# Orion-AI-Lab/KuroSiwo

Hardware: AMD Instinct MI355X
Metric: SAR tiles/sec (224x224, SNUNet-ECAM change-detection train step) (higher is better)
Workload: dtype bf16; 1 GPU; BASELINE.json configs[1]: SNUNet-ECAM CD, 2 dates x 2-ch GRD 224x224, per-GPU batch 32, ce+dice loss, Adam lr 1e-3, fwd+loss+bwd+optimizer; global_batch=32, base_channel=32, parallelism=dp1, hip_streams=3

## Files before the change

include/ksmi.h:

```cpp
#ifndef KSMI_H
#define KSMI_H
#include <stddef.h>
#include <stdint.h>

#ifdef __cplusplus
extern "C" {
#endif

#define KSMI_ABI_VERSION 8
#define KSMI_F32 0
#define KSMI_BF16 1
#define KSMI_E_ARG (-1)
#define KSMI_E_UNSUPPORTED (-2)
#define KSMI_MAX_SRC 6
#define KSMI_MAX_CHUNKS 72

int ksmi_abi_version(void);
const char* ksmi_last_error(void);
int ksmi_set_knob(const char* name, const char* value);
int ksmi_chunk_elems(int dtype);

#define KSMI_OP_CALL 0
#define KSMI_OP_ORDER 1
#define KSMI_OP_WAIT_SIDE 2
// ... 28 lines not shown
  int32_t C;
  int32_t c_off;
  int32_t n_begin;
  int32_t n_len;
  int32_t accumulate;
  int32_t pad_;
} ksmi_dst;

typedef struct ksmi_conv_desc {
  ksmi_src src[KSMI_MAX_SRC];
  ksmi_dst dst[KSMI_MAX_SRC];
  int32_t nsrc, ndst;
  const void* wpk;
  const float* bias;
  float* stats;
  const void* mask_src;
  const float* m_mean; const float* m_rstd; const float* m_scale; const float* m_shift;
  int32_t B, Hin, Win, Hout, Wout;
  int32_t KH, KW, stride, pad;
  int32_t TH, TW;
  int32_t N, Npad;
  int32_t nchunks;
  int32_t ps_cout;
  uint16_t chunk_c0[KSMI_MAX_CHUNKS];
  uint8_t chunk_src[KSMI_MAX_CHUNKS];
  int32_t pad_x;
  int32_t out_sy, out_sx, out_oy, out_ox, out_H, out_W;
  int32_t uniform_kc;
  int32_t in_sy, in_sx, in_oy, in_ox, in_H, in_W;
  float alpha;
  int32_t relu_out;
  int32_t residC;
  const void* resid;
  int32_t stats_rows;
  const void* gate_src; const void* xhat_src; const float* g_mean; const float* g_rstd;
  int32_t dir;
  int32_t pad2_;
} ksmi_conv_desc;


int ksmi_last_kernels(char* buf, int cap);
int ksmi_hbm_probe(int mode, const void* a, void* b, void* c, size_t nbytes, unsigned* sink, void* stream);
size_t ksmi_desc_size(int which);
int ksmi_conv_gate_supported(const ksmi_conv_desc* d, int dtype);
int ksmi_conv_grid_m(const ksmi_conv_desc* d);
int ksmi_conv_stats_rows(const ksmi_conv_desc* d, int dtype);
// ... 370 lines not shown
```

kurosiwo_amd/_lib.py:

```python
import ctypes as C
import os

_HERE = os.path.dirname(os.path.abspath(__file__))
LIB_PATH = os.path.join(_HERE, "libksmi.so")

KSMI_F32, KSMI_BF16 = 0, 1
LOSS_DICE, LOSS_LOVASZ, LOSS_FOCAL = 1, 2, 3
MAX_SRC, MAX_CHUNKS = 6, 72
ABI_VERSION = 8


class KsmiError(RuntimeError):
    pass


class Src(C.Structure):
    _fields_ = [("ptr", C.c_void_p), ("scale", C.c_void_p), ("shift", C.c_void_p),
                ("C", C.c_int32), ("c_off", C.c_int32), ("c_len", C.c_int32), ("relu", C.c_int32)]


class Dst(C.Structure):
    _fields_ = [("ptr", C.c_void_p), ("C", C.c_int32), ("c_off", C.c_int32), ("n_begin", C.c_int32),
                ("n_len", C.c_int32), ("accumulate", C.c_int32), ("pad_", C.c_int32)]


class ConvDesc(C.Structure):
    _fields_ = [("src", Src * MAX_SRC), ("dst", Dst * MAX_SRC), ("nsrc", C.c_int32), ("ndst", C.c_int32),
                ("wpk", C.c_void_p), ("bias", C.c_void_p), ("stats", C.c_void_p),
                ("mask_src", C.c_void_p), ("m_mean", C.c_void_p), ("m_rstd", C.c_void_p),
                ("m_scale", C.c_void_p), ("m_shift", C.c_void_p),
                ("B", C.c_int32), ("Hin", C.c_int32), ("Win", C.c_int32), ("Hout", C.c_int32), ("Wout", C.c_int32),
                ("KH", C.c_int32), ("KW", C.c_int32), ("stride", C.c_int32), ("pad", C.c_int32),
                ("TH", C.c_int32), ("TW", C.c_int32), ("N", C.c_int32), ("Npad", C.c_int32),
                ("nchunks", C.c_int32), ("ps_cout", C.c_int32),
                ("chunk_c0", C.c_uint16 * MAX_CHUNKS), ("chunk_src", C.c_uint8 * MAX_CHUNKS),
                ("pad_x", C.c_int32), ("out_sy", C.c_int32), ("out_sx", C.c_int32), ("out_oy", C.c_int32),
                ("out_ox", C.c_int32), ("out_H", C.c_int32), ("out_W", C.c_int32),
                ("uniform_kc", C.c_int32), ("in_sy", C.c_int32), ("in_sx", C.c_int32), ("in_oy", C.c_int32), ("in_ox", C.c_int32),
                ("in_H", C.c_int32), ("in_W", C.c_int32), ("alpha", C.c_float), ("relu_out", C.c_int32), ("residC", C.c_int32),
                ("resid", C.c_void_p), ("stats_rows", C.c_int32),
                ("gate_src", C.c_void_p), ("xhat_src", C.c_void_p), ("g_mean", C.c_void_p), ("g_rstd", C.c_void_p),
                ("dir", C.c_int32), ("pad2_", C.c_int32)]


class PackDesc(C.Structure):
    _fields_ = [("w", C.c_void_p), ("out", C.c_void_p),
                ("nchunks", C.c_int32), ("taps", C.c_int32), ("N", C.c_int32), ("Npad", C.c_int32), ("n_mod", C.c_int32),
                ("sK", C.c_int64), ("sN", C.c_int64), ("sD", C.c_int64), ("sT", C.c_int64),
                ("flip", C.c_int32),
                ("k_off", C.c_int32 * MAX_CHUNKS), ("k_len", C.c_int32 * MAX_CHUNKS),
                ("use_tap_map", C.c_int32), ("tap_map", C.c_int32 * 16), ("uniform_kc", C.c_int32), ("k_total", C.c_int32)]


class TiffInfo(C.Structure):
    _fields_ = [(k, C.c_int32) for k in ("width", "height", "bands", "bits", "sample_format", "compression", "predictor", "tiled",
                                         "big_endian", "bigtiff", "has_geo", "has_nodata")] + [
        ("pixel_scale", C.c_double * 2), ("origin", C.c_double * 2), ("tie_pixel", C.c_double * 2), ("nodata", C.c_double)]
# ... 292 lines not shown
```

kurosiwo_amd/csrc/conv_api.hip:

```cpp
#include <stdint.h>
#include "../../include/ksmi.h"
#include "errors.h"
#include "igemm1.h"
#include "igemm3.h"
#include "igemm4.h"
#include "wgrad3.h"

namespace {

enum RowsRule { ROWS_AS_SET, ROWS_OF_KERNEL };
struct ConvRoute { int gen; ksmi_igemm3_geom_t g3; ksmi_igemm4_geom_t g4; };

ConvRoute conv_route(const ksmi_conv_desc* d, int dtype, RowsRule rule) {
  static const bool force_v1 = ksmi_knob_is_set("KSMI_IGEMM_V1");
  ConvRoute r = {};
  r.gen = 1;
  if (force_v1) return r;
  auto rows_ok = [&](int gx) { return rule == ROWS_OF_KERNEL || d->stats == nullptr || d->stats_rows == gx; };
  if (!d->gate_src && ksmi_igemm3_geom(d, dtype, &r.g3) && rows_ok(r.g3.gx)) r.gen = 3;
  else if (ksmi_igemm4_geom(d, dtype, &r.g4) && rows_ok(r.g4.gx)) r.gen = 4;
  else if (ksmi_igemm2_eligible(d, dtype)) r.gen = 2;
  return r;
}

ConvRoute conv_route_with_stats(const ksmi_conv_desc* d, int dtype, bool gate) {
  ksmi_conv_desc c = *d;
  if (!c.stats) c.stats = (float*)(uintptr_t)16;
  if (gate && !c.gate_src) { c.gate_src = (const void*)(uintptr_t)16; c.xhat_src = c.gate_src; c.g_mean = (const float*)(uintptr_t)16; c.g_rstd = c.g_mean; }
  return conv_route(&c, dtype, ROWS_OF_KERNEL);
}

enum { CORE_PATCH = 1, CORE_TOKEN1 = 2, CORE_GEMM2 = 3, CORE_WGRAD3 = 4 };
struct WgradRoute {
  int core, reducer;
  int bias;
  bool plain, direct;
  int nsplit;
  ksmi_igemm1_wgeom_t g1;
  int rps, bt;
  ksmi_wgrad3_geom_t g3;
};

bool token_eligible(const ksmi_wgrad_desc* d, int dtype) {
  static const bool generic = ksmi_knob_is_set("KSMI_WGRAD_GENERIC");
  return dtype == KSMI_BF16 && d->KH == 1 && d->KW == 1 && d->stride == 1 && d->pad == 0 && d->nsrc == 1 && d->src[0].scale == nullptr &&
         d->Hin == d->Hout && d->Win == d->Wout && (d->src[0].c_len % 8) == 0 && (d->N % 8) == 0 && d->N >= 64 && d->src[0].c_len >= 64 && !generic;
}

WgradRoute wgrad_route(const ksmi_wgrad_desc* d, int dtype) {
  WgradRoute r = {};
  ksmi_igemm1_wgrad_geom(d, dtype, &r.g1);
// ... 125 lines not shown
```

kurosiwo_amd/csrc/igemm4.hip:

```cpp
#include <stdlib.h>
#include <type_traits>
#include "common.h"
#include "../../include/ksmi.h"
#include "errors.h"
#include "igemm_epilogue.h"
#include "igemm4.h"
#include "dma.h"

namespace {

template <int N> __device__ __forceinline__ void vm_wait_c() {
  static_assert(N >= 0 && N < 64, "vmcnt field");
  asm volatile("s_waitcnt vmcnt(%0)" ::"n"(N) : "memory");
}

__device__ __attribute__((aligned(64))) unsigned char ig4_zero_page[64];
KSMI_DEVICE_SYMBOL_GETTER(ig4_zero, ig4_zero_page)

struct Ig4Args {
  ksmi_conv_desc d;
  uint32_t m_tw, m_hw, m_tx, m_ty;
  int th, tw;
  int hslot, nh, nhs;
  int tiles, gx, gy;
  int rot;
  int stagger;
  int dbg;
  const unsigned char* zero;
};

constexpr int IG4_NHMAX = 5;

__device__ __forceinline__ int swz_h(int hx) { return ((hx >> 2) & 1) << 1; }

template <int WM, int NF, bool AFF, int EPI, bool DBG = false, int DIR = 0, int ROT = 0, int NWV = 8, int KH = 3, int KW = 3>
__global__ __launch_bounds__(64 * NWV, NWV == 4 ? 2 : 1) void igemm4_kernel(const Ig4Args ka) {
  typedef bf16_t T;
  constexpr bool MASK = EPI == 1, GATE = EPI == 2;
  const ksmi_conv_desc& d = ka.d;
  constexpr int NT = 64 * NWV;
  constexpr int WN = NWV / WM;
  constexpr int BNW = 16 * NF;
  constexpr int BN = WN * BNW;
  constexpr int NG = NF / 2;
  static_assert((KH == 3 && KW == 3) || (KH == 2 && KW == 2 && ROT == 3), "taps");
  constexpr int WSLOT = KW * BN * 64;
  constexpr int WPIECES = WSLOT / 1024;
  constexpr int WK = (WPIECES + NWV - 1) / NWV;
  constexpr int NHM = NWV == 4 ? 6 : (WM == 4 ? 3 : IG4_NHMAX);
  constexpr int HSLOT = NHM * NT * 16;
  constexpr int nh = NHM;
  constexpr bool CHUNK = ROT == 3;
  constexpr int NHS = (NWV == 4 || (WM == 8 && NF == 4) || (CHUNK && WM == 8)) ? 2 : 3;
  constexpr bool DEEP = ROT == 2;
  static_assert(!DEEP || (!AFF && !DBG && NHS == 3 && NWV == 8 && BN <= 64), "deep weight ring: 32 / 64-column tiles with three halo slots");
  static_assert(!CHUNK || (!AFF && !DBG && NWV == 8 && (NF == 2 || KH == 2)), "chunk-granular schedule: the NF = 2 tiles and the 2 x 2 phase convolutions");
  constexpr int NWS = CHUNK ? 2 * KH : (DEEP ? 5 : 3);
  constexpr int nhs = NHS;
  extern __shared__ __attribute__((aligned(16))) unsigned char smem[];

  const int tid = threadIdx.x, lane = tid & 63;
// ... 162 lines not shown
  if (tid < BN) bias_tab[tid] = (d.bias && n0 + tid < d.N) ? d.bias[n0 + tid] : 0.f;
  const bool want_stats = d.stats != nullptr;
  const bool late = ka.stagger && wave >= NWV / 2;
  constexpr int LA = NHS - 1;

  auto tile_epilogue = [&](int t, f32x4 (&acc)[4][NF]) {
      {
        int b, oy0, ox0;
        tile_origin(t, b, oy0, ox0);
        uint32_t opix[4];
        bool okp[4];
#pragma unroll
        for (int mf = 0; mf < 4; ++mf) {
          const int p = wm * 64 + mf * 16 + l15;
          const int ly = dTW.div(p), lx = p - ly * TW;
          const int oy = oy0 + ly, ox = ox0 + lx;
          okp[mf] = p < P && oy < d.Hout && ox < d.Wout;
          opix[mf] = (KH != 2 || d.out_sy == 0) ? (uint32_t)((b * d.Hout + oy) * d.Wout + ox)
                                                : (uint32_t)((b * d.out_H + (oy * d.out_sy + d.out_oy)) * d.out_W + (ox * d.out_sx + d.out_ox));
        }
#pragma unroll
        for (int gi = 0; gi < NG; ++gi) {
          const int nc = n0 + (wn * NG + gi) * 32 + g * 8;
          const bool nv = nc < d.N;
          T* const obase = (T*)d.dst[0].ptr + d.dst[0].c_off + nc;
          const T* const mbase = (const T*)d.mask_src + nc;
          float bias8[8], ssum[8], ssq[8];
          {
            const f32x4 a = *(const f32x4*)(bias_tab + (wn * NG + gi) * 32 + g * 8), c = *(const f32x4*)(bias_tab + (wn * NG + gi) * 32 + g * 8 + 4);
#pragma unroll
            for (int j = 0; j < 4; ++j) { bias8[j] = a[j]; bias8[4 + j] = c[j]; }
#pragma unroll
            for (int j = 0; j < 8; ++j) { ssum[j] = 0.f; ssq[j] = 0.f; }
          }
          float mm[(MASK || GATE) ? 8 : 1], mr[(MASK || GATE) ? 8 : 1], mg[MASK ? 8 : 1], mb[MASK ? 8 : 1];
          if constexpr (MASK || GATE) {
            auto ld8 = [&](const float* qp, float* o, int at) {
              const f32x4 a = *(const f32x4*)(qp + at), c = *(const f32x4*)(qp + at + 4);
#pragma unroll
              for (int j = 0; j < 4; ++j) { o[j] = a[j]; o[4 + j] = c[j]; }
            };
#pragma unroll
            for (int j = 0; j < 8; ++j) { mm[j] = 0.f; mr[j] = 0.f; }
            if constexpr (MASK) {
#pragma unroll
              for (int j = 0; j < 8; ++j) { mg[j] = 0.f; mb[j] = 0.f; }
              if (nv) { ld8(d.m_mean, mm, nc); ld8(d.m_rstd, mr, nc); ld8(d.m_scale, mg, nc); ld8(d.m_shift, mb, nc); }
            } else {
              if (nv) { ld8(d.g_mean, mm, nc); ld8(d.g_rstd, mr, nc); }
            }
          }
#pragma unroll
          for (int mh = 0; mh < 4; mh += 2) {
            u32x4 mv[2], zv[2], ov[2];
#pragma unroll
            for (int u = 0; u < 2; ++u) {
              const int mf = mh + u;
              mv[u] = (u32x4){0u, 0u, 0u, 0u}; zv[u] = mv[u]; ov[u] = mv[u];
              if constexpr (MASK) { if (nv && okp[mf]) mv[u] = *(const u32x4*)(mbase + (size_t)opix[mf] * d.N); }
              if constexpr (EPI == 0) { if (has_resid && nv && okp[mf]) mv[u] = *(const u32x4*)((const T*)d.resid + nc + (size_t)opix[mf] * d.residC); }
              if constexpr (GATE) {
                if (nv && okp[mf]) {
                  mv[u] = *(const u32x4*)((const T*)d.gate_src + nc + (size_t)opix[mf] * d.N);
                  zv[u] = *(const u32x4*)((const T*)d.xhat_src + nc + (size_t)opix[mf] * d.N);
                }
              }
              if (accum && nv && okp[mf]) ov[u] = *(const u32x4*)(obase + (size_t)opix[mf] * dC);
            }
#pragma unroll
            for (int u = 0; u < 2; ++u) {
              const int mf = mh + u;
              const bool ok = nv && okp[mf];
              float v[8];
#pragma unroll
              for (int r = 0; r < 4; ++r) { v[r] = acc[mf][2 * gi][r] + bias8[r]; v[4 + r] = acc[mf][2 * gi + 1][r] + bias8[4 + r]; }
              if constexpr (EPI == 0) {
                float rs[8];
                vec_unpack<T>(mv[u], rs);
#pragma unroll
                for (int j = 0; j < 8; ++j) {
                  v[j] = v[j] * alpha + rs[j];
                  if (relu_out) v[j] = fmaxf(v[j], 0.f);
                }
              }
              if constexpr (GATE) {
                float o[8], m[8], z[8];
                vec_unpack<T>(ov[u], o); vec_unpack<T>(mv[u], m); vec_unpack<T>(zv[u], z);
#pragma unroll
                for (int j = 0; j < 8; ++j) {
                  if (accum) v[j] += o[j];
                  if (!(m[j] > 0.f)) v[j] = 0.f;
                }
                const u32x4 pk = vec_pack<T>(v);
                float vr[8];
                vec_unpack<T>(pk, vr);
#pragma unroll
                for (int j = 0; j < 8; ++j) if (ok) { ssum[j] += vr[j]; ssq[j] += vr[j] * ((z[j] - mm[j]) * mr[j]); }
                if (ok && !(DBG && (dbg & 4))) *(u32x4*)(obase + (size_t)opix[mf] * dC) = pk;
              } else {
                if constexpr (MASK) {
                  float m[8];
                  vec_unpack<T>(mv[u], m);
#pragma unroll
                  for (int j = 0; j < 8; ++j) {
                    const float xh = (m[j] - mm[j]) * mr[j];
                    if (!(m[j] * mg[j] + mb[j] > 0.f)) v[j] = 0.f;
                    const float q = ElemTraits<T>::cvt(v[j]);
                    if (ok) { ssum[j] += q; ssq[j] += q * xh; }
                  }
                } else {
                  float q[8];
                  vec_unpack<T>(vec_pack<T>(v), q);
#pragma unroll
                  for (int j = 0; j < 8; ++j) if (ok) { ssum[j] += q[j]; ssq[j] += q[j] * q[j]; }
                }
                if (accum) {
                  float o[8];
                  vec_unpack<T>(ov[u], o);
#pragma unroll
                  for (int j = 0; j < 8; ++j) v[j] += o[j];
                }
// ... 447 lines not shown
      const int hp = (th + 2) * (tw + 2);
      if (hp > hmax) continue;
      const int tiles = ((H + th - 1) / th) * ((W + tw - 1) / tw);
      const double cost = (double)tiles * pmax * (1.0 + 0.15 * hp / pmax);
      if (cost < best) { best = cost; bth = th; btw = tw; }
    }
  *th_o = bth; *tw_o = btw;
}
}

bool ksmi_igemm4_geom(const ksmi_conv_desc* d, int dtype, ksmi_igemm4_geom_t* g) {
  static const bool off = ksmi_knob_is_set("KSMI_IGEMM4_OFF");
  if (off || dtype != KSMI_BF16) return false;
  static const int k2_on = ksmi_knob_int("KSMI_IG4_K2", 1);
  const bool k2 = d->KH == 2 && d->KW == 2;
  if (k2) {
    if (!k2_on || d->stride != 1 || (unsigned)d->pad > 1u || (unsigned)d->pad_x > 1u) return false;
    if (d->Npad % 128 || d->src[0].scale || d->gate_src || (d->out_sy && (d->mask_src || d->dst[0].accumulate))) return false;
    if (d->alpha != 0.f || d->resid || d->relu_out) return false;
  } else if (d->KH != 3 || d->KW != 3 || d->stride != 1 || d->pad != 1 || d->pad_x != 1) return false;
  if (d->Hin != d->Hout || d->Win != d->Wout) return false;
  if (d->nchunks < 2) return false;
  if (d->nchunks > KSMI_MAX_CHUNKS) return false;
  if (d->ndst != 1 || d->dst[0].n_begin != 0) return false;
  if (((d->out_sy || d->in_sy) && !k2) || d->ps_cout) return false;
  if (d->out_sy && ((size_t)d->B * d->out_H * d->out_W >= ((size_t)1 << 31))) return false;
  if ((d->alpha != 0.f || d->resid || d->relu_out) && (d->mask_src || d->gate_src)) return false;
  if (d->resid && (((uintptr_t)d->resid & 15) || (d->residC % 8))) return false;
  if ((d->dst[0].C % 8) || (d->dst[0].c_off % 8)) return false;
  static const int thin_on = ksmi_knob_int("KSMI_IG4_THIN", 1);
  if ((d->N % 8) && (!thin_on || k2 || d->mask_src || d->gate_src || d->resid || d->dst[0].accumulate || d->alpha != 0.f || d->relu_out ||
                     d->dst[0].c_off + ((d->N + 7) & ~7) > d->dst[0].C)) return false;
  if (d->Npad != 32 && (d->Npad % 64)) return false;
  auto al16 = [](const void* q) { return ((uintptr_t)q & 15) == 0; };
  if (!al16(d->dst[0].ptr) || !al16(d->bias) || !al16(d->mask_src) || !al16(d->m_mean) || !al16(d->m_rstd) || !al16(d->m_scale) || !al16(d->m_shift))
    return false;
  for (int i = 0; i < d->nsrc; ++i) {
    if (d->src[i].c_len % 32) return false;
    if (d->src[i].scale && (i > 0 || d->nsrc != 1)) return false;
    if (!al16(d->src[i].ptr) || (d->src[i].C % 8) || (d->src[i].c_off % 8)) return false;
    const size_t ipx = d->in_sy ? (size_t)d->B * d->in_H * d->in_W : (size_t)d->B * d->Hin * d->Win;
    if (ipx * (size_t)d->src[i].C * 2 >= ((size_t)1 << 32)) return false;
  }
  if ((size_t)d->B * d->Hout * d->Wout >= ((size_t)1 << 31)) return false;
  const bool aff = d->src[0].scale != nullptr;
  if (aff && (d->mask_src || d->gate_src)) return false;
  if (d->mask_src && d->gate_src) return false;
// ... 24 lines not shown
    int th, tw;
    if (wm == 4) { th = d->TH; tw = d->TW; if (th * tw > 256) continue; }
    else {
      ig4_patch(d->Hout, d->Wout, 512, IG4_NHMAX * 128, &th, &tw);
      char pe[32];
      int pth = 0, ptw = 0;
      if (ksmi_knob_str("KSMI_IG4_PATCH", pe, sizeof(pe)) && sscanf(pe, "%d,%d", &pth, &ptw) == 2 && pth > 0 && ptw > 0 && pth * ptw <= 512 && (pth + 2) * (ptw + 2) <= IG4_NHMAX * 128) { th = pth; tw = ptw; }
    }
    const int hp = (th + d->KH - 1) * (tw + d->KW - 1);
    const int tilesX = (d->Wout + tw - 1) / tw, tilesY = (d->Hout + th - 1) / th;
    const int tiles = d->B * tilesX * tilesY;
    const int gy = d->Npad / bn;
    if (!wm_force && tiles < 64) continue;
    if (!wm_force && ci + 1 < nc && (size_t)tiles * gy < 192) continue;
    g->WM = wm; g->NF = nf; g->nwv = nwv; g->th = th; g->tw = tw;
    g->tiles = tiles; g->gy = gy;
    g->nh = nwv == 4 ? 6 : (wm == 4 ? 3 : IG4_NHMAX);
    g->hslot = g->nh * nwv * 1024;
    if (hp * 64 > g->hslot) continue;
    const size_t tabs = (size_t)(nwv * 2 * 16 * nf + bn) * 4 + (size_t)KSMI_MAX_CHUNKS * 16 + (aff ? (size_t)d->nchunks * 32 * 2 * 4 : 0);
    static const int rot_on = ksmi_knob_int("KSMI_IG4_ROT", 1);
    static const int deep_on = ksmi_knob_int("KSMI_IG4_DEEP", 0);
    static const int chunk_on = ksmi_knob_int("KSMI_IG4_CHUNK", 0);
    const bool chunk = k2 || (rot_on && chunk_on && !aff && nwv == 8 && nf == 2);
    const int nhs_ = (nwv == 4 || (wm == 8 && nf == 4) || (chunk && wm == 8)) ? 2 : 3;
    const bool deep = !chunk && rot_on && deep_on && !aff && nhs_ == 3 && nwv == 8 && nf == 2;
    g->deep = chunk ? 2 : (deep ? 1 : 0);
    const size_t wr = (chunk ? 2 * d->KH : (deep ? 5 : 3)) * (size_t)(d->KW * bn * 64);
    g->nhs = nhs_;
    g->lds = (size_t)g->nhs * g->hslot + wr + ((d->KW * bn / 16) % nwv ? 4096 : 0) + tabs;
    const int per_cu = nwv == 4 ? 2 : 1;
    if (g->lds * per_cu > 160 * 1024) continue;
    int gx = cus * per_cu / gy;
    if (gx < 1) gx = 1;
    if (gx > tiles) gx = tiles;
    const int rounds = (tiles + gx - 1) / gx;
    gx = (tiles + rounds - 1) / rounds;
    if (gx >= 8 && ((gx + 7) / 8 * 8) * gy <= (cus > 8 ? cus : 8) * per_cu) gx = (gx + 7) / 8 * 8;
    g->gx = gx;
    return true;
  }
  return false;
}

static thread_local bool ig4_dry = false;
#define KSMI_IG4_DRY_RETURN do { if (ig4_dry) return 0; } while (0)

bool ksmi_igemm4_launchable(const ksmi_conv_desc* d, const ksmi_igemm4_geom_t* g) {
  ig4_dry = true;
// ... 46 lines not shown
  } while (0)
#define KSMI_G4V(WM_, NF_)                                                                           \
  do { if (ka.rot) { if (aff) KSMI_G4R(WM_, NF_, true, 0); else if (mask) KSMI_G4R(WM_, NF_, false, 1); else if (gate) KSMI_G4R(WM_, NF_, false, 2); else KSMI_G4R(WM_, NF_, false, 0); } \
       if (aff) KSMI_G4(WM_, NF_, true, 0); else if (mask) KSMI_G4(WM_, NF_, false, 1); else if (gate) KSMI_G4(WM_, NF_, false, 2);   \
       else if (d->dir == 1) KSMI_G4D(WM_, NF_); else KSMI_G4(WM_, NF_, false, 0); } while (0)
  if (ka.dbg && !aff && !mask && !gate && g->NF == 2 && g->WM == 8 && g->nwv == 8) {
    auto kfn = igemm4_kernel<8, 2, false, 0, true>; KSMI_IG4_DRY_RETURN; KSMI_NOTE(kfn);
    (void)hipFuncSetAttribute((const void*)kfn, hipFuncAttributeMaxDynamicSharedMemorySize, 160 * 1024);
    hipLaunchKernelGGL(kfn, grid, dim3(512), g->lds, st, ka);
    return ksmi_check_launch("igemm4");
  }
  if (ka.dbg && !aff && !mask && !gate && g->NF == 4 && g->nwv == 8) {
    if (g->WM == 4) {
      auto kfn = igemm4_kernel<4, 4, false, 0, true>; KSMI_IG4_DRY_RETURN; KSMI_NOTE(kfn);
      (void)hipFuncSetAttribute((const void*)kfn, hipFuncAttributeMaxDynamicSharedMemorySize, 160 * 1024);
      hipLaunchKernelGGL(kfn, grid, dim3(512), g->lds, st, ka);
    } else {
      auto kfn = igemm4_kernel<8, 4, false, 0, true>; KSMI_IG4_DRY_RETURN; KSMI_NOTE(kfn);
      (void)hipFuncSetAttribute((const void*)kfn, hipFuncAttributeMaxDynamicSharedMemorySize, 160 * 1024);
      hipLaunchKernelGGL(kfn, grid, dim3(512), g->lds, st, ka);
    }
    return ksmi_check_launch("igemm4");
  }
  if (g->nwv == 4) {
#define KSMI_G4N(AFF_, EPI_, ROT_)                                                                   \
  do {                                                                                               \
    auto kfn = igemm4_kernel<4, 2, AFF_, EPI_, false, 0, ROT_ ? 1 : 0, 4>; KSMI_IG4_DRY_RETURN; KSMI_NOTE(kfn);                           \
    static bool attr_set = false;                                                                    \
    if (!attr_set) { (void)hipFuncSetAttribute((const void*)kfn, hipFuncAttributeMaxDynamicSharedMemorySize, 80 * 1024); attr_set = true; } \
    hipLaunchKernelGGL(kfn, grid, dim3(256), g->lds, st, ka);                                        \
    return ksmi_check_launch("igemm4");                                                              \
  } while (0)
    if (g->WM != 4 || g->NF != 2) return ksmi_fail(KSMI_E_UNSUPPORTED, "igemm4: no 4-wave instance");
    if (ka.rot) { if (aff) KSMI_G4N(true, 0, true); else if (mask) KSMI_G4N(false, 1, true); else if (gate) KSMI_G4N(false, 2, true); else KSMI_G4N(false, 0, true); }
    if (aff) KSMI_G4N(true, 0, false); else if (mask) KSMI_G4N(false, 1, false); else if (gate) KSMI_G4N(false, 2, false); else KSMI_G4N(false, 0, false);
#undef KSMI_G4N
  }
  if (g->deep == 2 && d->KH == 2) {
#define KSMI_G4K2(EPI_)                                                                              \
  do {                                                                                               \
    auto kfn = igemm4_kernel<4, 4, false, EPI_, false, 0, 3, 8, 2, 2>; KSMI_IG4_DRY_RETURN; KSMI_NOTE(kfn);                               \
    static bool attr_set = false;                                                                    \
    if (!attr_set) { (void)hipFuncSetAttribute((const void*)kfn, hipFuncAttributeMaxDynamicSharedMemorySize, 160 * 1024); attr_set = true; } \
    hipLaunchKernelGGL(kfn, grid, dim3(512), g->lds, st, ka);                                        \
    return ksmi_check_launch("igemm4");                                                              \
  } while (0)
// ... 43 lines not shown
```

kurosiwo_amd/functional.py:

```python
import ctypes as C

import torch

from . import _lib
from .runtime import DT, SrcSpec, conv_grid_m, conv_npad, conv_stats_rows, make_conv, make_pack, make_wgrad, packed_weight_numel, require_gpu, stream_ptr


def to_nhwc(x_nchw, dtype):
    require_gpu(x_nchw)
    B, Cc, H, W = x_nchw.shape
    y = torch.empty((B, H, W, Cc), dtype=dtype, device=x_nchw.device)
    _lib.check(_lib.load().ksmi_nchw_to_nhwc(x_nchw.contiguous().float().data_ptr(), y.data_ptr(), B, Cc, H * W, DT[dtype], stream_ptr()))
    return y


def to_nchw(x_nhwc):
    B, H, W, Cc = x_nhwc.shape
    y = torch.empty((B, Cc, H, W), dtype=torch.float32, device=x_nhwc.device)
    _lib.check(_lib.load().ksmi_nhwc_to_nchw(x_nhwc.data_ptr(), y.data_ptr(), B, Cc, H * W, DT[x_nhwc.dtype], stream_ptr()))
    return y


def _pack(weight, table, taps, N, n_mod, sK, sN, sD, sT, flip, dtype):
    Npad = conv_npad(N)
# ... 8 lines not shown
    dtype = xs[0].dtype
    B, H, W, _ = xs[0].shape
    N = weight.shape[0]
    Ktot = sum(x.shape[3] for x in xs)
    srcs = [SrcSpec(x, x.shape[3]) for x in xs]
    if affine is not None:
        srcs[0].scale, srcs[0].shift, srcs[0].relu = affine
    if out is None:
        out = torch.empty((B, H, W, N), dtype=dtype, device=xs[0].device)
    d, table = make_conv(srcs, [(out, out.shape[3], 0, 0, N, accumulate)], out, bias, None, B, H, W, H, W, 3, 3, 1, 1, N, dtype,
                         alpha=alpha, relu_out=relu_out, resid=None if resid is None else (resid, resid.shape[3]), mask=mask)
    wpk = _pack(weight.contiguous(), table, 9, N, N, 9, Ktot * 9, 0, 1, 0, dtype)
    d.wpk = wpk.data_ptr()
    if gate is not None:
        d.gate_src, d.xhat_src, d.g_mean, d.g_rstd = (t.data_ptr() for t in gate)
        if not _lib.load().ksmi_conv_gate_supported(C.byref(d), DT[dtype]):
            raise _lib.KsmiError("conv3x3: the gate epilogue is not available for this shape")
    stats = None
    if want_stats:
        stats = torch.zeros((conv_stats_rows(d, dtype), 2, d.Npad), dtype=torch.float32, device=out.device)
        d.stats = stats.data_ptr()
    _lib.check(_lib.load().ksmi_conv_forward(C.byref(d), DT[dtype], stream_ptr()), "conv_forward")
    return out, stats


def conv3x3_dgrad(dy, weight, splits):
    dtype = dy.dtype
    B, H, W, N = dy.shape
    Ktot = sum(splits)
    outs = [torch.empty((B, H, W, c), dtype=dtype, device=dy.device) for c in splits]
    dsts, nb = [], 0
    for o, c in zip(outs, splits):
        dsts.append((o, c, 0, nb, c, 0))
        nb += c
    d, table = make_conv([SrcSpec(dy, N)], dsts, dy, None, None, B, H, W, H, W, 3, 3, 1, 1, Ktot, dtype)
    wpk = _pack(weight.contiguous(), table, 9, Ktot, Ktot, Ktot * 9, 9, 0, 1, 1, dtype)
    d.wpk = wpk.data_ptr()
    _lib.check(_lib.load().ksmi_conv_forward(C.byref(d), DT[dtype], stream_ptr()), "conv_dgrad")
    return outs


def conv3x3_wgrad(xs, dy, affine=None, n_real=None):
    dtype = dy.dtype
    B, H, W, dyC = dy.shape
    N = dyC if n_real is None else n_real
    Ktot = sum(x.shape[3] for x in xs)
# ... 300 lines not shown
```

kurosiwo_amd/snunet_plan.py:

```python
import ctypes as C
import os

import torch

from . import _lib
from .plan_base import PlanBase, _Saved
from .runtime import Act, SrcSpec, conv_npad, conv_stats_rows, make_conv, make_pack, make_wgrad, packed_weight_numel
from .snunet import BN_EPS, BN_MOMENTUM


class SNUNetPlan(PlanBase):
    side_wgrad = True
    two_lanes = True
    bn_fused = os.environ.get("KSMI_BN_FUSED", "1") != "0"
    im2col_late = os.environ.get("KSMI_IM2COL_LATE", "1") != "0"
    up_gemm = os.environ.get("KSMI_UP_GEMM", "1") != "0"
    up_wgrad64 = os.environ.get("KSMI_UP_WGRAD64", "1") != "0"
    up_wgrad128 = os.environ.get("KSMI_UP_WGRAD128", "1") != "0"
    pack_kind = "pack_weights_batched"

    def __init__(self, model, B, H, W, dtype, training, with_backward, tail=0, sync_bn=False):
        self._init_lists(model, dtype, with_backward)
        self.B, self.H, self.W = B, H, W
        from . import distributed as _D
        self.sync_bn = bool(sync_bn) and training
        self.bn_world = _D.world_size() if self.sync_bn else 1
        if self.sync_bn:
            self.bn_fused = False
        self.training = training
        self._up_packs = []
        self._rowsums = []
        n, c = model.base_channel, model.in_channels
        self.n = n
        f = [n, 2 * n, 4 * n, 8 * n, 16 * n]
        self.tail = tail
        self.xA = torch.empty((B, c - tail, H, W), dtype=torch.float32, device=self.dev)
        self.xB = torch.empty_like(self.xA)
        self.xtail = torch.empty((B, tail, H, W), dtype=torch.float32, device=self.dev) if tail else None
        self.logits = torch.empty((B, 3, H, W), dtype=torch.float32, device=self.dev)
        self.dlogits = torch.empty_like(self.logits) if with_backward else None
        self.bwd_builders = []

        def A(name, lvl, ch):
            return Act(name, B, H >> lvl, W >> lvl, ch, dtype, self.dev)

        L = self._lane
        L(0); x0_0A, p0A = self._block("conv0_0", "A", [self.xA], A("x0_0A", 0, f[0]), first=True, pool="p0A")
        self._handover(0, 1, back=(1, 0))
        L(1); x0_0B, p0B = self._block("conv0_0", "B", [self.xB], A("x0_0B", 0, f[0]), first=True, pool="p0B")
        L(0); x1_0A, p1A = self._block("conv1_0", "A", [self._pool_at(x0_0A, p0A, "p0A")], A("x1_0A", 1, f[1]), pool="p1A")
        self._handover(0, 1, back=(1, 0))
        L(1); x1_0B, p1B = self._block("conv1_0", "B", [self._pool_at(x0_0B, p0B, "p0B")], A("x1_0B", 1, f[1]), pool="p1B")
        L(0); x2_0A, p2A = self._block("conv2_0", "A", [self._pool_at(x1_0A, p1A, "p1A")], A("x2_0A", 2, f[2]), pool="p2A")
        self._handover(0, 1, back=(1, 0))
        L(1); x2_0B, p2B = self._block("conv2_0", "B", [self._pool_at(x1_0B, p1B, "p1B")], A("x2_0B", 2, f[2]), pool="p2B")
        L(0); x3_0A = self._block("conv3_0", "A", [self._pool_at(x2_0A, p2A, "p2A")], A("x3_0A", 3, f[3]))
        self._handover(0, 1, back=(1, 0))
        L(1); x3_0B, p3B = self._block("conv3_0", "B", [self._pool_at(x2_0B, p2B, "p2B")], A("x3_0B", 3, f[3]), pool="p3B")
        x4_0B = self._block("conv4_0", "B", [self._pool_at(x3_0B, p3B, "p3B")], A("x4_0B", 4, f[4]))
        self._handover(1, 0, back=(0, 1))

        self._handover(0, 1, back=(1, 0))
        L(0); x0_1 = self._block("conv0_1", "", [x0_0A, x0_0B, self._up("Up1_0", x1_0B)], A("x0_1", 0, f[0]))
        L(1); x1_1 = self._block("conv1_1", "", [x1_0A, x1_0B, self._up("Up2_0", x2_0B)], A("x1_1", 1, f[1]))
# ... 123 lines not shown
            ch0 += nch
        d.wpk = wpk.data_ptr()
        self.keep.append(wpk)
        gated = None
        if gate is not None:
            g_out, g_z, g_sv = gate
            d.gate_src, d.xhat_src, d.g_mean, d.g_rstd = g_out.data_ptr(), g_z.data_ptr(), g_sv.mean, g_sv.rstd
            if self.lib.ksmi_conv_gate_supported(C.byref(d), self.dt):
                rows_g = conv_stats_rows(d, self.dtype)
                st = torch.empty(rows_g * 2 * Npad, dtype=torch.float32, device=self.dev)
                d.stats = st.data_ptr()
                self.keep.append(st)
                gated = (st, rows_g, Npad)
            else:
                d.gate_src = d.xhat_src = d.g_mean = d.g_rstd = None
        if bias_key is not None:
            rows_g = conv_stats_rows(d, self.dtype)
            st = torch.empty(rows_g * 2 * Npad, dtype=torch.float32, device=self.dev)
            d.stats = st.data_ptr()
            self._rowsum_at_end(bias_key, st, rows_g, 2, 0, Npad, Cc)
        self._conv(self.bwd, d, "dgrad")
        return gated if gated is not None else True

    def _pool(self, x, name):
        y = Act(name, x.B, x.H // 2, x.W // 2, x.C, self.dtype, self.dev)
        self._level(x.H)
        self.fwd.add("ksmi_maxpool2x2_forward", lambda: (x.t.data_ptr(), y.t.data_ptr(), x.B, x.H, x.W, x.C, self.dt))
        self._pool_bwd(x, y)
        return y

    def _pool_at(self, x, y, name):
        if y is None:
            return self._pool(x, name)
        self._pool_bwd(x, y)
        return y

    def _pool_bwd(self, x, y):
        def build_bwd():
            self._level(x.H)
            self._emit_dgrad(y)
            acc = x.take_acc_flag()
            gy, gx = y.grad(), x.grad()
            self.bwd.add("ksmi_maxpool2x2_backward", lambda: (x.t.data_ptr(), gy.data_ptr(), gx.data_ptr(), acc,
                                                              x.B, x.H, x.W, x.C, self.dt))
        self.bwd_builders.append((self.fwd.cur_lane, build_bwd))

# ... 129 lines not shown
        d2.wpk = w2.data_ptr()
        rows2 = conv_stats_rows(d2, dtype)
        if training:
            self.need(sS, rows2 * 2 * Npad * 4)
            self.patch(d2, "stats", sS)
        self._conv(self.fwd, d2)
        fused = training and self.bn_fused and bool(self.lib.ksmi_bn_fused_supported(Cc, Npad, dt))
        pooled = None
        if fused:
            if pool is not None:
                pooled = Act(pool, B, H // 2, W // 2, Cc, dtype, self.dev)
            nbt2 = m._c(f"{name}.bn2.num_batches_tracked").data_ptr()
            pp = pooled.t.data_ptr() if pooled is not None else None
            self.fwd.add("ksmi_bn_fin_add_relu", lambda: (stats(), rows2, Npad, Cc, float(npix), P("bn2.weight"), P("bn2.bias"),
                                                          Bf("bn2.running_mean"), Bf("bn2.running_var"), nbt2, BN_MOMENTUM, BN_EPS,
                                                          sv2.mean, sv2.rstd, sv2.scale, sv2.shift, z_act.t.data_ptr(), i_act.t.data_ptr(),
                                                          out.t.data_ptr(), pp, B, H, W, dt),
                         {"kind": "bn_fin_add_relu", "bytes": npix * Cc * self._es() * (3.25 if pooled is not None else 3), "flops": 0})
        else:
            bn_fin("bn2", sv2, rows2, Npad)
            self.fwd.add("ksmi_bn_add_relu", lambda: (z_act.t.data_ptr(), i_act.t.data_ptr(), sv2.scale, sv2.shift,
                                                      out.t.data_ptr(), npix, Cc, dt))

        def build_bwd():
            self._level(H)
            gated = self._emit_dgrad(out, gate=(out.t, z_act.t, sv2)) if os.environ.get("KSMI_NO_GATE") is None else self._emit_dgrad(out)
            gated = gated if isinstance(gated, tuple) else None
            rows = self._rows(npix)
            self.need(sR, rows * 2 * Cc * 4)
            sums1 = torch.zeros((2, Cc), dtype=torch.float32, device=self.dev)
            sums2 = torch.zeros((2, Cc), dtype=torch.float32, device=self.dev)
            dz = torch.empty_like(z_act.t)
            r = torch.empty_like(i_act.t)
            self.keep += [sums1, sums2, dz, r]
            gout = out.grad().data_ptr()
            s1p, s2p = sums1.data_ptr(), sums2.data_ptr()
            a_bn2 = self._acc_param(f"{name}.bn2")
            es = self._es()
            if gated is not None:
                gst, grows, gpad = gated
                if fused and self.lib.ksmi_bn_fused_supported(Cc, gpad, dt):
                    self.bwd.add("ksmi_bn_bwd_fin_apply_gated", lambda: (gst.data_ptr(), grows, gpad, s2p, G("bn2.weight"), G("bn2.bias"), a_bn2,
                                                                         gout, z_act.t.data_ptr(), sv2.mean, sv2.rstd, P("bn2.weight"),
                                                                         dz.data_ptr(), float(npix), npix, Cc, dt),
                                 {"kind": "bn_bwd_fin_apply_gated", "bytes": npix * Cc * es * 3, "flops": 0})
                    self._mark(f"{name}.bn2.weight", f"{name}.bn2.bias")
                else:
                    self.bwd.add("ksmi_reduce_rows", lambda: (gst.data_ptr(), grows, 2, gpad, Cc, s2p, G("bn2.weight"), G("bn2.bias"), a_bn2))
                    self._mark(f"{name}.bn2.weight", f"{name}.bn2.bias")
                    if self.sync_bn:
# ... 137 lines not shown
```

Baseline: 2240 tiles/s.

## Fuse paired encoder-branch dgrad convs into one two-destination gated igemm4 launch

The siamese encoder's two branches (A and B) feed the same downstream convs, so their input-gradient convolutions are merged into one 3x3 dgrad with 2*Cc output channels. The igemm4 kernel gains a PAIR epilogue that splits columns between two destination tensors, each with its own ReLU gate, xhat source and BN mean/rstd for the gated statistics. The goal is to halve the number of dgrad launches at each paired level and re-read the shared upstream gradient once instead of twice. In exchange it builds a separate packed weight layout, extends the descriptor ABI, and can add a cross-lane wait or fall back to the unpaired path when the lanes differ.

```diff
diff --git a/include/ksmi.h b/include/ksmi.h
--- a/include/ksmi.h
+++ b/include/ksmi.h
@@ -74,6 +74,7 @@
   int32_t N, Npad;
   int32_t nchunks;
   int32_t ps_cout;
+  const void* gate2_src; const void* xhat2_src; const float* g2_mean; const float* g2_rstd;
   uint16_t chunk_c0[KSMI_MAX_CHUNKS];
   uint8_t chunk_src[KSMI_MAX_CHUNKS];
   int32_t pad_x;
diff --git a/kurosiwo_amd/_lib.py b/kurosiwo_amd/_lib.py
--- a/kurosiwo_amd/_lib.py
+++ b/kurosiwo_amd/_lib.py
@@ -33,6 +33,7 @@
                 ("KH", C.c_int32), ("KW", C.c_int32), ("stride", C.c_int32), ("pad", C.c_int32),
                 ("TH", C.c_int32), ("TW", C.c_int32), ("N", C.c_int32), ("Npad", C.c_int32),
                 ("nchunks", C.c_int32), ("ps_cout", C.c_int32),
+                ("gate2_src", C.c_void_p), ("xhat2_src", C.c_void_p), ("g2_mean", C.c_void_p), ("g2_rstd", C.c_void_p),
                 ("chunk_c0", C.c_uint16 * MAX_CHUNKS), ("chunk_src", C.c_uint8 * MAX_CHUNKS),
                 ("pad_x", C.c_int32), ("out_sy", C.c_int32), ("out_sx", C.c_int32), ("out_oy", C.c_int32),
                 ("out_ox", C.c_int32), ("out_H", C.c_int32), ("out_W", C.c_int32),
diff --git a/kurosiwo_amd/csrc/conv_api.hip b/kurosiwo_amd/csrc/conv_api.hip
--- a/kurosiwo_amd/csrc/conv_api.hip
+++ b/kurosiwo_amd/csrc/conv_api.hip
@@ -27,6 +27,7 @@
   ksmi_conv_desc c = *d;
   if (!c.stats) c.stats = (float*)(uintptr_t)16;
   if (gate && !c.gate_src) { c.gate_src = (const void*)(uintptr_t)16; c.xhat_src = c.gate_src; c.g_mean = (const float*)(uintptr_t)16; c.g_rstd = c.g_mean; }
+  if (c.gate_src && c.ndst == 2 && !c.gate2_src) { c.gate2_src = c.gate_src; c.xhat2_src = c.gate_src; c.g2_mean = c.g_mean; c.g2_rstd = c.g_mean; }
   return conv_route(&c, dtype, ROWS_OF_KERNEL);
 }
 
diff --git a/kurosiwo_amd/csrc/igemm4.hip b/kurosiwo_amd/csrc/igemm4.hip
--- a/kurosiwo_amd/csrc/igemm4.hip
+++ b/kurosiwo_amd/csrc/igemm4.hip
@@ -36,7 +36,7 @@
 template <int WM, int NF, bool AFF, int EPI, bool DBG = false, int DIR = 0, int ROT = 0, int NWV = 8, int KH = 3, int KW = 3>
 __global__ __launch_bounds__(64 * NWV, NWV == 4 ? 2 : 1) void igemm4_kernel(const Ig4Args ka) {
   typedef bf16_t T;
-  constexpr bool MASK = EPI == 1, GATE = EPI == 2;
+  constexpr bool MASK = EPI == 1, GATE = EPI == 2 || EPI == 3, PAIR = EPI == 3;
   const ksmi_conv_desc& d = ka.d;
   constexpr int NT = 64 * NWV;
   constexpr int WN = NWV / WM;
@@ -245,8 +245,15 @@
 #pragma unroll
         for (int gi = 0; gi < NG; ++gi) {
           const int nc = n0 + (wn * NG + gi) * 32 + g * 8;
-          const bool nv = nc < d.N;
-          T* const obase = (T*)d.dst[0].ptr + d.dst[0].c_off + nc;
+          const bool second = PAIR && n0 + (wn * NG + gi) * 32 >= d.dst[1].n_begin;
+          const int ncl = PAIR ? (second ? nc - d.dst[1].n_begin : nc) : nc;
+          const int gC = PAIR ? (second ? d.dst[1].n_len : d.dst[0].n_len) : d.N;
+          const bool nv = PAIR ? ncl < gC : nc < d.N;
+          const int dCk = PAIR ? (second ? d.dst[1].C : dC) : dC;
+          const bool accum_k = PAIR ? (second ? d.dst[1].accumulate != 0 : accum) : accum;
+          T* const obase = (PAIR && second) ? (T*)d.dst[1].ptr + d.dst[1].c_off + ncl : (T*)d.dst[0].ptr + d.dst[0].c_off + nc;
+          const T* const gsrc = (const T*)((PAIR && second) ? d.gate2_src : d.gate_src);
+          const T* const zsrc = (const T*)((PAIR && second) ? d.xhat2_src : d.xhat_src);
           const T* const mbase = (const T*)d.mask_src + nc;
           float bias8[8], ssum[8], ssq[8];
           {
@@ -270,7 +277,7 @@
               for (int j = 0; j < 8; ++j) { mg[j] = 0.f; mb[j] = 0.f; }
               if (nv) { ld8(d.m_mean, mm, nc); ld8(d.m_rstd, mr, nc); ld8(d.m_scale, mg, nc); ld8(d.m_shift, mb, nc); }
             } else {
-              if (nv) { ld8(d.g_mean, mm, nc); ld8(d.g_rstd, mr, nc); }
+              if (nv) { ld8((PAIR && second) ? d.g2_mean : d.g_mean, mm, ncl); ld8((PAIR && second) ? d.g2_rstd : d.g_rstd, mr, ncl); }
             }
           }
 #pragma unroll
@@ -284,11 +291,11 @@
               if constexpr (EPI == 0) { if (has_resid && nv && okp[mf]) mv[u] = *(const u32x4*)((const T*)d.resid + nc + (size_t)opix[mf] * d.residC); }
               if constexpr (GATE) {
                 if (nv && okp[mf]) {
-                  mv[u] = *(const u32x4*)((const T*)d.gate_src + nc + (size_t)opix[mf] * d.N);
-                  zv[u] = *(const u32x4*)((const T*)d.xhat_src + nc + (size_t)opix[mf] * d.N);
+                  mv[u] = *(const u32x4*)(gsrc + ncl + (size_t)opix[mf] * gC);
+                  zv[u] = *(const u32x4*)(zsrc + ncl + (size_t)opix[mf] * gC);
                 }
               }
-              if (accum && nv && okp[mf]) ov[u] = *(const u32x4*)(obase + (size_t)opix[mf] * dC);
+              if (accum_k && nv && okp[mf]) ov[u] = *(const u32x4*)(obase + (size_t)opix[mf] * dCk);
             }
 #pragma unroll
             for (int u = 0; u < 2; ++u) {
@@ -311,7 +318,7 @@
                 vec_unpack<T>(ov[u], o); vec_unpack<T>(mv[u], m); vec_unpack<T>(zv[u], z);
 #pragma unroll
                 for (int j = 0; j < 8; ++j) {
-                  if (accum) v[j] += o[j];
+                  if (accum_k) v[j] += o[j];
                   if (!(m[j] > 0.f)) v[j] = 0.f;
                 }
                 const u32x4 pk = vec_pack<T>(v);
@@ -319,7 +326,7 @@
                 vec_unpack<T>(pk, vr);
 #pragma unroll
                 for (int j = 0; j < 8; ++j) if (ok) { ssum[j] += vr[j]; ssq[j] += vr[j] * ((z[j] - mm[j]) * mr[j]); }
-                if (ok && !(DBG && (dbg & 4))) *(u32x4*)(obase + (size_t)opix[mf] * dC) = pk;
+                if (ok && !(DBG && (dbg & 4))) *(u32x4*)(obase + (size_t)opix[mf] * dCk) = pk;
               } else {
                 if constexpr (MASK) {
                   float m[8];
@@ -813,7 +820,17 @@
   if (d->Hin != d->Hout || d->Win != d->Wout) return false;
   if (d->nchunks < 2) return false;
   if (d->nchunks > KSMI_MAX_CHUNKS) return false;
-  if (d->ndst != 1 || d->dst[0].n_begin != 0) return false;
+  const bool pair = d->ndst == 2;
+  if ((d->ndst != 1 && !pair) || d->dst[0].n_begin != 0) return false;
+  if (pair) {
+    static const int pair_on = ksmi_knob_int("KSMI_IG4_PAIR", 1);
+    const ksmi_dst &a = d->dst[0], &b = d->dst[1];
+    if (!pair_on || k2 || !d->gate_src || !d->gate2_src || d->mask_src || d->src[0].scale || d->bias) return false;
+    if (b.n_begin <= 0 || (b.n_begin % 32) || a.n_len != b.n_begin || b.n_len <= 0 || b.n_begin + b.n_len != d->N || (d->N % 8)) return false;
+    if (a.c_off || b.c_off || a.C != a.n_len || b.C != b.n_len || (b.C % 8)) return false;
+    if (!d->xhat2_src || !d->g2_mean || !d->g2_rstd) return false;
+    if (((uintptr_t)b.ptr | (uintptr_t)d->gate2_src | (uintptr_t)d->xhat2_src | (uintptr_t)d->g2_mean | (uintptr_t)d->g2_rstd) & 15) return false;
+  }
   if (((d->out_sy || d->in_sy) && !k2) || d->ps_cout) return false;
   if (d->out_sy && ((size_t)d->B * d->out_H * d->out_W >= ((size_t)1 << 31))) return false;
   if ((d->alpha != 0.f || d->resid || d->relu_out) && (d->mask_src || d->gate_src)) return false;
@@ -884,9 +901,9 @@
     static const int rot_on = ksmi_knob_int("KSMI_IG4_ROT", 1);
     static const int deep_on = ksmi_knob_int("KSMI_IG4_DEEP", 0);
     static const int chunk_on = ksmi_knob_int("KSMI_IG4_CHUNK", 0);
-    const bool chunk = k2 || (rot_on && chunk_on && !aff && nwv == 8 && nf == 2);
+    const bool chunk = k2 || (rot_on && chunk_on && !aff && !pair && nwv == 8 && nf == 2);
     const int nhs_ = (nwv == 4 || (wm == 8 && nf == 4) || (chunk && wm == 8)) ? 2 : 3;
-    const bool deep = !chunk && rot_on && deep_on && !aff && nhs_ == 3 && nwv == 8 && nf == 2;
+    const bool deep = !chunk && rot_on && deep_on && !aff && !pair && nhs_ == 3 && nwv == 8 && nf == 2;
     g->deep = chunk ? 2 : (deep ? 1 : 0);
     const size_t wr = (chunk ? 2 * d->KH : (deep ? 5 : 3)) * (size_t)(d->KW * bn * 64);
     g->nhs = nhs_;
@@ -979,6 +996,15 @@
     }
     return ksmi_check_launch("igemm4");
   }
+  if (d->ndst == 2) {
+    if (!gate || g->nwv != 8 || g->deep) return ksmi_fail(KSMI_E_UNSUPPORTED, "igemm4: no two-destination instance");
+#define KSMI_G4P(WM_, NF_) do { if (ka.rot) KSMI_G4R(WM_, NF_, false, 3); KSMI_G4(WM_, NF_, false, 3); } while (0)
+    if (g->WM == 4 && g->NF == 4) KSMI_G4P(4, 4);
+    if (g->WM == 4 && g->NF == 2) KSMI_G4P(4, 2);
+    if (g->WM == 8 && g->NF == 4) KSMI_G4P(8, 4);
+#undef KSMI_G4P
+    return ksmi_fail(KSMI_E_UNSUPPORTED, "igemm4: no two-destination instance");
+  }
   if (g->nwv == 4) {
 #define KSMI_G4N(AFF_, EPI_, ROT_)                                                                   \
   do {                                                                                               \
diff --git a/kurosiwo_amd/functional.py b/kurosiwo_amd/functional.py
--- a/kurosiwo_amd/functional.py
+++ b/kurosiwo_amd/functional.py
@@ -54,6 +54,28 @@
         d.stats = stats.data_ptr()
     _lib.check(_lib.load().ksmi_conv_forward(C.byref(d), DT[dtype], stream_ptr()), "conv_forward")
     return out, stats
+
+
+def conv3x3_gate_pair(xs, weight, outs, accumulate, gates):
+    dtype = xs[0].dtype
+    B, H, W, _ = xs[0].shape
+    N = weight.shape[0]
+    C0, C1 = outs[0].shape[3], outs[1].shape[3]
+    assert C0 + C1 == N
+    Ktot = sum(x.shape[3] for x in xs)
+    srcs = [SrcSpec(x, x.shape[3]) for x in xs]
+    d, table = make_conv(srcs, [(outs[0], C0, 0, 0, C0, accumulate[0]), (outs[1], C1, 0, C0, C1, accumulate[1])], outs[0], None, None,
+                         B, H, W, H, W, 3, 3, 1, 1, N, dtype)
+    wpk = _pack(weight.contiguous(), table, 9, N, N, 9, Ktot * 9, 0, 1, 0, dtype)
+    d.wpk = wpk.data_ptr()
+    d.gate_src, d.xhat_src, d.g_mean, d.g_rstd = (t.data_ptr() for t in gates[0])
+    d.gate2_src, d.xhat2_src, d.g2_mean, d.g2_rstd = (t.data_ptr() for t in gates[1])
+    if not _lib.load().ksmi_conv_gate_supported(C.byref(d), DT[dtype]):
+        raise _lib.KsmiError("conv3x3_gate_pair: the two-destination gate epilogue is not available for this shape")
+    stats = torch.zeros((conv_stats_rows(d, dtype), 2, d.Npad), dtype=torch.float32, device=outs[0].device)
+    d.stats = stats.data_ptr()
+    _lib.check(_lib.load().ksmi_conv_forward(C.byref(d), DT[dtype], stream_ptr()), "conv_forward")
+    return outs, stats
 
 
 def conv3x3_dgrad(dy, weight, splits):
diff --git a/kurosiwo_amd/snunet_plan.py b/kurosiwo_amd/snunet_plan.py
--- a/kurosiwo_amd/snunet_plan.py
+++ b/kurosiwo_amd/snunet_plan.py
@@ -40,6 +40,11 @@
         self.logits = torch.empty((B, 3, H, W), dtype=torch.float32, device=self.dev)
         self.dlogits = torch.empty_like(self.logits) if with_backward else None
         self.bwd_builders = []
+        self.pair_dgrad = os.environ.get("KSMI_NO_PAIR") is None and os.environ.get("KSMI_NO_GATE") is None
+        self.pair_all = os.environ.get("KSMI_PAIR_ALL", "0") == "1"
+        self._pair_a = {}
+        self._pair_done = {}
+        self.paired_levels = []
 
         def A(name, lvl, ch):
             return Act(name, B, H >> lvl, W >> lvl, ch, dtype, self.dev)
@@ -209,6 +214,50 @@
         self._conv(self.bwd, d, "dgrad")
         return gated if gated is not None else True
 
+    def _emit_dgrad_pair(self, act_a, gate_a, act_b, gate_b):
+        ca, cb = getattr(act_a, "consumers", []), getattr(act_b, "consumers", [])
+        Cc = act_a.C
+        if not ca or len(ca) != len(cb) or act_b.C != Cc or Cc % 32:
+            return None
+        for (ra, ja, wa, oa, ka), (rb, jb, wb, ob, kb) in zip(ca, cb):
+            if ra is not rb or ja != jb or wa != wb or ka != kb or ob != oa + Cc:
+                return None
+        B, H, W = act_a.B, act_a.H, act_a.W
+        srcs = [SrcSpec(r, cj) for (r, cj, _, _, _) in ca]
+        d, table = make_conv(srcs, [(act_a.grad(), Cc, 0, 0, Cc, 0), (act_b.grad(), Cc, 0, Cc, Cc, 0)], act_a.grad(), None, None,
+                             B, H, W, H, W, 3, 3, 1, 1, 2 * Cc, self.dtype)
+        d.gate_src, d.xhat_src, d.g_mean, d.g_rstd = gate_a[0].data_ptr(), gate_a[1].data_ptr(), gate_a[2].mean, gate_a[2].rstd
+        d.gate2_src, d.xhat2_src, d.g2_mean, d.g2_rstd = gate_b[0].data_ptr(), gate_b[1].data_ptr(), gate_b[2].mean, gate_b[2].rstd
+        if not self.lib.ksmi_conv_gate_supported(C.byref(d), self.dt):
+            return None
+        needs_edge = act_a.ginit and self.bwd.cur_lane != 0
+        if needs_edge and not self.pair_all:
+            return None
+        d.dst[0].accumulate, d.dst[1].accumulate = act_a.take_acc_flag(), act_b.take_acc_flag()
+        Npad = conv_npad(2 * Cc)
+        wpk = torch.empty(packed_weight_numel(table, 9, Npad, self.dtype), dtype=self.dtype, device=self.dev)
+        kc = 32 if self.dtype == torch.bfloat16 else 16
+        slab = 9 * Npad * kc
+        ch0 = 0
+        for (r, cj, wkey, coff, ktot) in ca:
+            nch = -(-cj // kc)
+            tj = [(0, c0, c0, min(kc, cj - c0)) for c0 in range(0, cj, kc)]
+            wview = self.m._p(wkey)[coff * 9:]
+            out = wpk[ch0 * slab:(ch0 + nch) * slab]
+            pd = make_pack(wview, out, tj, 9, 2 * Cc, Npad, 2 * Cc, ktot * 9, 9, 0, 1, 1)
+            self.keep += [pd, wview, out]
+            self._pack_descs.append(pd)
+            ch0 += nch
+        d.wpk = wpk.data_ptr()
+        rows_g = conv_stats_rows(d, self.dtype)
+        st = torch.empty(rows_g * 2 * Npad, dtype=torch.float32, device=self.dev)
+        d.stats = st.data_ptr()
+        self.keep += [wpk, st]
+        if needs_edge:
+            self.bwd.add_wait(0, self.bwd.cur_lane)
+        self._conv(self.bwd, d, "dgrad")
+        return st, rows_g, Npad
+
     def _pool(self, x, name):
         y = Act(name, x.B, x.H // 2, x.W // 2, x.C, self.dtype, self.dev)
         self._level(x.H)
@@ -384,10 +433,23 @@
             self.fwd.add("ksmi_bn_add_relu", lambda: (z_act.t.data_ptr(), i_act.t.data_ptr(), sv2.scale, sv2.shift,
                                                       out.t.data_ptr(), npix, Cc, dt))
 
+        if branch == "A" and self.pair_dgrad and not self.sync_bn:
+            self._pair_a[name] = (out, (out.t, z_act.t, sv2))
+
         def build_bwd():
             self._level(H)
-            gated = self._emit_dgrad(out, gate=(out.t, z_act.t, sv2)) if os.environ.get("KSMI_NO_GATE") is None else self._emit_dgrad(out)
-            gated = gated if isinstance(gated, tuple) else None
+            gated = None
+            if branch == "B" and name in self._pair_a:
+                pair = self._emit_dgrad_pair(*self._pair_a[name], out, (out.t, z_act.t, sv2))
+                if pair is not None:
+                    self._pair_done[name] = pair
+                    self.paired_levels.append(name)
+                    gated = (pair[0][Cc:], pair[1], pair[2])
+            elif branch == "A" and name in self._pair_done:
+                gated = self._pair_done[name]
+            if gated is None:
+                gated = self._emit_dgrad(out, gate=(out.t, z_act.t, sv2)) if os.environ.get("KSMI_NO_GATE") is None else self._emit_dgrad(out)
+                gated = gated if isinstance(gated, tuple) else None
             rows = self._rows(npix)
             self.need(sR, rows * 2 * Cc * 4)
             sums1 = torch.zeros((2, Cc), dtype=torch.float32, device=self.dev)
```

Measured after the change: 2230 tiles/s. Within noise of the previous version (-0.4%).
